# AKGWSB/EzRT

Measured on NVIDIA H100. Metric: Mrays/s (primary+secondary), higher is better.
Workload: dtype f32

## Files before the change

### ezrt_b200/_lib.py

```python
import ctypes as C
import os

from . import build as _build

c_float_p = C.POINTER(C.c_float)
c_int32_p = C.POINTER(C.c_int32)
c_uint32_p = C.POINTER(C.c_uint32)


class RenderParams(C.Structure):
    _fields_ = [
        ("width", C.c_int32), ("height", C.c_int32), ("spp", C.c_int32), ("first_frame", C.c_uint32),
        ("max_bounce", C.c_int32), ("mode", C.c_int32),
        ("eye", C.c_float * 3), ("camera_rotate", C.c_float * 16), ("env_color", C.c_float * 3),
        ("traverse", C.c_int32), ("pipeline", C.c_int32), ("out_channels", C.c_int32),
        ("part_rank", C.c_int32), ("part_count", C.c_int32), ("frames_per_batch", C.c_int32),
        ("profile", C.c_int32), ("reserved", C.c_int32 * 3),
    ]


class AdaptiveParams(C.Structure):
    _fields_ = [("threshold", C.c_float), ("min_spp", C.c_int32), ("check_interval", C.c_int32), ("reserved", C.c_int32)]


# ... 7 lines not shown
                ("reserved", C.c_int32)]


class Counters(C.Structure):
    _fields_ = [
        ("rays", C.c_uint64), ("primary_rays", C.c_uint64), ("bounce_rays", C.c_uint64), ("shadow_rays", C.c_uint64),
        ("samples", C.c_uint64), ("kernel_launches", C.c_uint64), ("device_ms", C.c_double),
        ("deferred_rays", C.c_uint64), ("node_visits", C.c_uint64), ("tri_tests", C.c_uint64), ("node_visits_96", C.c_uint64),
        ("node_bytes", C.c_uint64), ("tri_bytes", C.c_uint64),
    ]


SIGNATURES = {
    "ezrt_last_error": (C.c_char_p, []),
    "ezrt_version": (C.c_int, []),
    "ezrt_scene_create": (C.c_int, [C.c_int, c_float_p, C.c_int, c_float_p, C.c_int, c_float_p, c_float_p, C.c_int, C.c_int,
                                    C.c_int, C.POINTER(C.c_void_p)]),
    "ezrt_scene_destroy": (C.c_int, [C.c_void_p]),
    "ezrt_scene_set_medium": (C.c_int, [C.c_void_p, C.POINTER(Medium)]),
    "ezrt_render": (C.c_int, [C.c_void_p, C.POINTER(RenderParams), c_float_p]),
    "ezrt_render_device": (C.c_int, [C.c_void_p, C.POINTER(RenderParams), C.c_void_p, C.c_void_p]),
    "ezrt_render_adaptive_device": (C.c_int, [C.c_void_p, C.POINTER(RenderParams), C.POINTER(AdaptiveParams), C.c_void_p, C.c_void_p,
                                              C.c_void_p, C.c_void_p]),
    "ezrt_render_adaptive": (C.c_int, [C.c_void_p, C.POINTER(RenderParams), C.POINTER(AdaptiveParams), c_float_p, c_int32_p, c_float_p]),
    "ezrt_render_aov_device": (C.c_int, [C.c_void_p, C.POINTER(RenderParams), C.c_void_p, C.c_void_p, C.c_void_p, C.c_void_p]),
    "ezrt_render_aov": (C.c_int, [C.c_void_p, C.POINTER(RenderParams), c_float_p, c_float_p, c_float_p]),
    "ezrt_denoise_device": (C.c_int, [C.c_void_p, C.POINTER(DenoiseParams), C.c_void_p, C.c_int, C.c_void_p, C.c_void_p, C.c_int, C.c_int,
                                      C.c_int, C.c_void_p, C.c_void_p]),
    "ezrt_denoise": (C.c_int, [C.c_void_p, C.POINTER(DenoiseParams), c_float_p, C.c_int, c_float_p, c_float_p, C.c_int, C.c_int, C.c_int,
                               c_float_p]),
    "ezrt_get_counters": (C.c_int, [C.c_void_p, C.POINTER(Counters)]),
    "ezrt_get_kernel_times": (C.c_int, [C.c_void_p, C.POINTER(C.c_double), C.POINTER(C.c_uint64)]),
    "ezrt_get_w8_phase_cycles": (C.c_int, [C.c_void_p, C.POINTER(C.c_uint64)]),
    "ezrt_partition_pixels": (C.c_int64, [C.c_int, C.c_int, C.c_int, C.c_int]),
    "ezrt_partition_scatter": (C.c_int, [C.c_void_p, C.c_void_p, C.c_int, C.c_int, C.c_int, C.c_int, C.c_int, C.c_void_p]),
    "ezrt_partition_cache_clear": (C.c_int, [C.c_int]),
    "ezrt_host_sort_is_reference": (C.c_int, []),
    "ezrt_accel_build": (C.c_int, [C.c_int, c_float_p, C.c_int, C.c_int, C.c_int, c_int32_p, c_float_p, C.c_int, c_uint32_p, C.POINTER(C.c_double)]),
    "ezrt_partition_scatter_host": (C.c_int, [c_float_p, c_float_p, C.c_int, C.c_int, C.c_int, C.c_int, C.c_int]),
    "ezrt_trace_rays": (C.c_int, [C.c_void_p, C.c_int, c_float_p, c_float_p, C.c_int, C.c_int, C.c_int, c_int32_p, c_float_p,
                                  c_int32_p, c_int32_p, c_float_p, c_float_p]),
    "ezrt_scene_lights": (C.c_int, [C.c_void_p, C.c_int, c_int32_p, c_float_p, C.POINTER(C.c_double)]),
    "ezrt_scene_env_light": (C.c_int, [C.c_void_p, c_float_p, c_float_p, c_float_p, C.POINTER(C.c_double)]),
    "ezrt_occluded_rays": (C.c_int, [C.c_void_p, C.c_int, c_float_p, c_float_p, c_float_p, C.c_int, c_int32_p]),
    "ezrt_eval_brdf": (C.c_int, [C.c_int, C.c_int, C.c_int, c_float_p, c_float_p, c_float_p, c_float_p, c_float_p, c_float_p]),
    "ezrt_eval_bsdf": (C.c_int, [C.c_int, C.c_int, C.c_int, c_float_p, c_float_p, c_float_p, c_float_p, c_int32_p, c_float_p, c_float_p]),
    "ezrt_camera_rays": (C.c_int, [C.c_void_p, C.POINTER(RenderParams), C.c_int, c_uint32_p, c_uint32_p, c_uint32_p, c_float_p, c_float_p]),
    "ezrt_eval_math": (C.c_int, [C.c_int, C.c_int, C.c_int, c_float_p, c_float_p, c_float_p]),
    "ezrt_post_tonemap": (C.c_int, [C.c_void_p, C.c_int, C.c_void_p, C.c_int64, C.c_float, C.c_void_p]),
    "ezrt_write_png": (C.c_int, [C.c_char_p, c_float_p, C.c_int, C.c_int, C.c_int, C.c_int]),
    "ezrt_trilist_create": (C.c_void_p, []),
    "ezrt_trilist_destroy": (None, [C.c_void_p]),
    "ezrt_trilist_size": (C.c_int, [C.c_void_p]),
    "ezrt_transform_matrix": (None, [c_float_p, c_float_p, c_float_p, c_float_p]),
    "ezrt_trilist_read_obj": (C.c_int, [C.c_void_p, C.c_char_p, c_float_p, c_float_p, C.c_int]),
    "ezrt_trilist_read_obj_text": (C.c_int, [C.c_void_p, C.c_char_p, C.c_size_t, c_float_p, c_float_p, C.c_int]),
    "ezrt_trilist_append_encoded": (C.c_int, [C.c_void_p, c_float_p, C.c_int]),
    "ezrt_trilist_build_bvh": (C.c_int, [C.c_void_p, C.c_int, C.c_int]),
    "ezrt_trilist_node_count": (C.c_int, [C.c_void_p]),
    "ezrt_trilist_encode_triangles": (C.c_int, [C.c_void_p, c_float_p]),
    "ezrt_trilist_encode_nodes": (C.c_int, [C.c_void_p, c_float_p]),
    "ezrt_scene_file_load": (C.c_int, [C.c_char_p, C.c_void_p, c_float_p, C.c_char_p, C.c_size_t]),
    "ezrt_hdr_load": (C.c_int, [C.c_char_p, C.POINTER(C.c_int), C.POINTER(C.c_int), c_float_p]),
    "ezrt_hdr_cache": (C.c_int, [c_float_p, C.c_int, C.c_int, c_float_p]),
    "ezrt_hdr_cache_device": (C.c_int, [C.c_int, c_float_p, C.c_int, C.c_int, c_float_p, C.POINTER(C.c_double)]),
    "ezrt_camera_orbit": (None, [C.c_float, C.c_float, C.c_float, c_float_p, c_float_p]),
# ... 38 lines not shown
```

### ezrt_b200/api.py

```python
import ctypes as C
from dataclasses import dataclass, field

import numpy as np

from . import _lib
from ._lib import AdaptiveParams, Counters, DenoiseParams, EzrtError, Medium, RenderParams, check, lib

MODE_DIFFUSE_P3 = 0
MODE_DISNEY_ANISO_P4 = 1
MODE_DISNEY_SOBOL_P5 = 2
MODE_DISNEY_IS_MIS_P5 = 3
MODE_DISNEY_LIGHTS = 4
PARAM_ACCUMULATE = 1
PARAM_ENV_LIGHT = 2
PARAM_TRANSMISSION = 4
PARAM_THIN_LENS = 8
PARAM_MEDIUM = 16
MODES = {"diffuse_p3": 0, "disney_aniso_p4": 1, "disney_sobol_p5": 2, "disney_is_mis_p5": 3, "disney_lights": 4}

TRAVERSE_ACCEL = 0
TRAVERSE_REFERENCE = 1
TRAVERSE_PRUNED = 2
PIPELINE_WAVEFRONT = 0
PIPELINE_MEGAKERNEL = 1
# ... 325 lines not shown
        feat, m2 = _f32(aov, (h, w, AOV_CHANNELS)), _f32(luma2, (h, w))
        if out is None:
            out = np.empty_like(img)
        assert out.dtype == np.float32 and out.shape == img.shape and out.flags.c_contiguous
        d = denoise_params(**{**DENOISE_DEFAULTS, **sigmas})
        check(lib.ezrt_denoise(self._h, C.byref(d), _fp(img), ch, _fp(feat), _fp(m2), w, h, int(n), _fp(out)))
        return out

    def denoise_device(self, d_image, channels, d_aov, d_luma2, width, height, n, d_out, stream=None, **sigmas):
        ptr = lambda t: t.data_ptr() if hasattr(t, "data_ptr") else int(t)
        st = 0 if stream is None else (stream.cuda_stream if hasattr(stream, "cuda_stream") else int(stream))
        d = denoise_params(**{**DENOISE_DEFAULTS, **sigmas})
        check(lib.ezrt_denoise_device(self._h, C.byref(d), C.c_void_p(ptr(d_image)), int(channels), C.c_void_p(ptr(d_aov)),
                                      C.c_void_p(ptr(d_luma2)), int(width), int(height), int(n), C.c_void_p(ptr(d_out)), C.c_void_p(st)))
        return d_out

    def counters(self):
        c = Counters()
        check(lib.ezrt_get_counters(self._h, C.byref(c)))
        return c

    def kernel_times(self):
        ms = (C.c_double * 4)()
        n = (C.c_uint64 * 4)()
        check(lib.ezrt_get_kernel_times(self._h, ms, n))
        return {k: (ms[i], int(n[i])) for i, k in enumerate(("extend", "shade", "shadow", "other"))}

    def w8_phase_cycles(self):
        c = (C.c_uint64 * 8)()
        check(lib.ezrt_get_w8_phase_cycles(self._h, c))
        phases = ("refill", "node", "triangle", "ray_end")
        return {k: {ph: int(c[4 * i + j]) for j, ph in enumerate(phases)} for i, k in enumerate(("k_extend_w8", "k_shadow_w8"))}

    def trace_rays(self, origins, dirs, traverse=TRAVERSE_ACCEL, any_hit=False, p3_normal_fudge=False):
        o = _f32(origins, (-1, 3))
        d = _f32(dirs, (-1, 3))
        n = o.shape[0]
        hit = np.zeros(n, dtype=np.int32); tri = np.zeros(n, dtype=np.int32); inside = np.zeros(n, dtype=np.int32)
        dist = np.zeros(n, dtype=np.float32); point = np.zeros((n, 3), dtype=np.float32); normal = np.zeros((n, 3), dtype=np.float32)
        ip = lambda a: a.ctypes.data_as(_lib.c_int32_p)
        check(lib.ezrt_trace_rays(self._h, n, _fp(o), _fp(d), int(traverse), int(bool(any_hit)), int(bool(p3_normal_fudge)),
                                  ip(hit), _fp(dist), ip(tri), ip(inside), _fp(point), _fp(normal)))
        return dict(hit=hit, distance=dist, triangle=tri, inside=inside, point=point, normal=normal)

    def camera_rays(self, cfg, px, py, frame):
        u = lambda a: np.ascontiguousarray(a, dtype=np.uint32).reshape(-1)
        px, py, frame = u(px), u(py), u(frame)
        n = px.size
        assert py.size == n and frame.size == n
        o, d = np.zeros((n, 3), np.float32), np.zeros((n, 3), np.float32)
        p = cfg.to_struct()
        up = lambda a: a.ctypes.data_as(_lib.c_uint32_p)
        check(lib.ezrt_camera_rays(self._h, C.byref(p), n, up(px), up(py), up(frame), _fp(o), _fp(d)))
        return o, d

    def lights(self):
        k = check(lib.ezrt_scene_lights(self._h, 0, None, None, None))
        tri = np.zeros(k, np.int32)
        cdf = np.zeros(k, np.float32)
        total = C.c_double(0.0)
        check(lib.ezrt_scene_lights(self._h, k, tri.ctypes.data_as(_lib.c_int32_p), _fp(cdf), C.byref(total)))
        return tri, cdf, total.value

    def env_light_table(self):
        total = C.c_double(0.0)
        if not check(lib.ezrt_scene_env_light(self._h, None, None, None, C.byref(total))):
# ... 78 lines not shown
```

### ezrt_b200/csrc/accel_w8.cpp

```cpp
#include <math.h>
#include <sched.h>
#include <stdio.h>
#include <stdlib.h>
#include <string.h>

#include <algorithm>
#include <atomic>
#include <chrono>
#include <thread>
#include <utility>
#include <vector>

#include "ezrt_internal.h"
#include "w8_node.h"

namespace {

inline float box_area(const EzrtAccelNode& c) {
    const float x = c.BB[0] - c.AA[0], y = c.BB[1] - c.AA[1], z = c.BB[2] - c.AA[2];
    return x * y + x * z + y * z;
}

}

// ... 138 lines not shown
    Pick stack[32];
    int sp = 0;
    stack[sp++] = {n0, k0};
    while (sp > 0) {
        Pick p = stack[--sp];
        const float* c = &C[(size_t)p.n * 8];
        while (p.k > 1 && c[p.k] == c[p.k - 1]) p.k--;
        if (p.k == 1 || a[p.n].n > 0) { roots[cnt++] = p.n; continue; }
        const EzrtAccelNode& nd = a[p.n];
        const float *cl = &C[(size_t)nd.left * 8], *cr = &C[(size_t)nd.right * 8];
        int bk = 1;
        float best = 3.0e38f;
        for (int k = 1; k < p.k; k++)
            if (cl[k] + cr[p.k - k] < best) { best = cl[k] + cr[p.k - k]; bk = k; }
        stack[sp++] = {nd.right, p.k - bk};
        stack[sp++] = {nd.left, bk};
    }
    return cnt;
}

int EzrtCollapse::children(int b, int* ch) const {
    const std::vector<EzrtAccelNode>& a = *an;
    const EzrtAccelNode& nd = a[b];
    const float *cl = &C[(size_t)nd.left * 8], *cr = &C[(size_t)nd.right * 8];
    int bk = 1;
    float best = 3.0e38f;
    for (int k = 1; k <= width - 1; k++)
        if (cl[k] + cr[width - k] < best) { best = cl[k] + cr[width - k]; bk = k; }
    int cnt = collect(nd.left, bk, ch);
    cnt += collect(nd.right, width - bk, ch + cnt);
    return cnt;
}

#define W8_COST_NODE 1.0
#define W8_COST_TRI 0.4

int ezrt_build_w8(const std::vector<EzrtAccelNode>& an, const std::vector<uint32_t>& order_in, float pad, float max_abs_coord,
                  const int axis_bit[3], EzrtW8Tree& out) {
    out.nodes.clear();
    out.tri_order.clear();
    out.leaf_first.assign(an.size(), -1);
    out.depth = 0;
    out.n_nodes = 0;
    out.n_children = 0;
    if (an.empty()) return -1;
    const int NB = (int)an.size();
    const double min_step = (double)max_abs_coord * (double)W8_MIN_STEP_REL;
    EzrtCollapse col;
    const int crc = col.build(an, 8, W8_MAX_LEAF_TRIS, W8_COST_NODE, W8_COST_TRI);
    if (crc) return crc;
    const std::vector<int>& first = col.first;
    const std::vector<int>& count = col.count;
    const std::vector<char>& as_leaf = col.as_leaf;

    struct Item { int bnode, level; };
    std::vector<Item> queue;
    queue.push_back({0, 1});
    out.tri_order.reserve(order_in.size());
    std::vector<int> new_pos(order_in.size(), -1);
    for (size_t wi = 0; wi < queue.size(); wi++) {
        const int b = queue[wi].bnode, level = queue[wi].level;
        out.depth = std::max(out.depth, level);
        int ch[8];
        int cnt = 0;
        if (an[b].n > 0 || (wi == 0 && as_leaf[b])) {
            ch[cnt++] = b;
        } else {
            cnt = col.children(b, ch);
        }
        double nlo[3] = {3.0e38, 3.0e38, 3.0e38}, nhi[3] = {-3.0e38, -3.0e38, -3.0e38};
        for (int k = 0; k < cnt; k++)
            for (int a = 0; a < 3; a++) {
                nlo[a] = std::min(nlo[a], (double)an[ch[k]].AA[a] - (double)pad);
                nhi[a] = std::max(nhi[a], (double)an[ch[k]].BB[a] + (double)pad);
            }
        int slot_child[8];
        for (int s = 0; s < 8; s++) slot_child[s] = -1;
        {
            double cost[8][8];
            for (int k = 0; k < cnt; k++)
                for (int s = 0; s < 8; s++) {
                    double c = 0.0;
// ... 340 lines not shown
```

### ezrt_b200/csrc/capi.cu

```cuda
#include <cuda_runtime.h>

#include <chrono>
#include <cmath>
#include <cstdio>
#include <cstdlib>
#include <cstring>
#include <functional>
#include <array>
#include <map>
#include <mutex>
#include <new>
#include <string>
#include <thread>
#include <vector>

#include "device_scene.h"
#include "ezrt.h"
#include "ezrt_internal.h"
#include "ezrt_math.h"
#include "kernels.h"
#include "w8_node.h"

#define CU_CHECK(call)                                                                                  \
    do {                                                                                                \
// ... 531 lines not shown
            return ezrt_set_error(EZRT_ERR_CUDA, "scene_create: upload failed: %s", cudaGetErrorString(cudaGetLastError()));
    }
    lap("triangles: upload");
    EzrtPrepInfo prep;
    {
        int r = sc->tri_geo.ensure((size_t)n_triangles * 4 * sizeof(float4));
        if (!r) r = sc->tri_shade.ensure((size_t)n_triangles * 3 * sizeof(float4));
        if (!r) r = ezrt_prep_records((const float*)raw.p, n_triangles, sc->tri_geo.p, sc->tri_shade.p, prep);
        if (r) return r;
    }
    std::vector<float4> mats;
    for (int m = 0; m < prep.n_materials; m++) {
        const float* v = &prep.materials[(size_t)m * EZRT_MATERIAL_FLOATS];
        mats.push_back(make_float4(v[0], v[1], v[2], v[3]));
        mats.push_back(make_float4(v[4], v[5], v[6], v[7]));
        mats.push_back(make_float4(v[8], v[9], v[10], v[11]));
        mats.push_back(make_float4(v[12], v[13], v[14], v[15]));
        mats.push_back(make_float4(v[16], v[17], 0.0f, 0.0f));
    }
    const float max_abs = prep.max_abs;
    float bmin[3], bmax[3];
    for (int k = 0; k < 3; k++) { bmin[k] = prep.bmin[k]; bmax[k] = prep.bmax[k]; }
    lap("triangles: geometry / shading records, materials (device)");
    const float prune_delta = max_abs * 1.52587890625e-05f;
    EzrtW4Tree w4;
    EzrtRawArray<float>& acc_wide = w4.nodes;
    EzrtRawArray<uint32_t>& acc_wide_q = w4.q16;
    std::vector<uint32_t> w8_words;
    int acc_wide_root = 0;
    std::vector<uint32_t> acc_order;
    int acc_depth = 0, w8_depth = 0, w8_near_bit[3] = {0, 1, 2};
    bool have_accel = true;
    {
        std::vector<EzrtAccelNode> an;
        std::vector<uint32_t> order_bin;
        const char* be = getenv("EZRT_BUILD");
        if (be && !strcmp(be, "host")) {
            ezrt_build_accel(tris, n_triangles, W8_MAX_LEAF_TRIS, an, order_bin);
            lap("acceleration tree: binary SAH build (host)");
        } else {
            const int brc = ezrt_build_accel_device((const float*)raw.p, n_triangles, W8_MAX_LEAF_TRIS, an, order_bin, nullptr);
            if (brc < 0) return brc;
            lap("acceleration tree: binary SAH build (device)");
        }
        const float pad = 2.0f * prune_delta;
        int accel_form = (n_triangles >= (1 << 16)) ? 8 : 4;
        if (const char* we = getenv("EZRT_ACCEL")) {
            const int v = atoi(we);
            if (v == 4 || v == 8) accel_form = v;
        }
        if (an[0].n > 0) accel_form = 8;
        EzrtW8Tree w8;
        ezrt_w8_axis_bits(bmin, bmax, w8_near_bit);
        if (accel_form == 8) {
            const int wrc = ezrt_build_w8(an, order_bin, pad, max_abs, w8_near_bit, w8);
            if (wrc != 0 || w8.depth > EZRT_W8_SMEM_STACK + W8_LOCAL_STACK) {
                have_accel = false;
            } else {
                acc_order = w8.tri_order;
                w8_words.swap(w8.nodes);
                w8_depth = w8.depth;
            }
        } else {
            const char* ce = getenv("EZRT_W4_COLLAPSE");
            const bool greedy = ce && !strcmp(ce, "greedy");
            const char* qe = getenv("EZRT_ACCEL_Q16");
            const bool want_q16 = !(qe && atoi(qe) == 0);
            if (ezrt_build_w4(an, pad, max_abs, greedy, want_q16, ezrt_host_threads(), w4) != 0) {
                have_accel = false;
            } else {
                acc_order = order_bin;
                acc_wide_root = w4.root;
                acc_depth = w4.depth;
                if (3 * w4.depth + 2 > EZRT_ACCEL_STACK) { w4.nodes.clear(); have_accel = false; }
                if (!have_accel) w4.q16.clear();
            }
        }
        if (!have_accel) {
            acc_order.resize(n_triangles);
            for (int i = 0; i < n_triangles; i++) acc_order[i] = (uint32_t)i;
        }
        raw.release();
    }
    lap("acceleration tree: collapse, pack");
    if (guard.worker.joinable()) guard.worker.join();
    if (verbose) fprintf(stderr, "[ezrt_scene_create] %-44s %8.1f ms (worker thread, overlapped)\n", "reference tree: decode, validate, repack", ref_ms);
    if (ref_rc) return ezrt_set_error(ref_rc, "%s", ref_msg.c_str());
    lap("wait for the reference-tree worker");
// ... 672 lines not shown
    CU_CHECK(cudaMemcpyAsync(d_aov, aov, sizeof(float) * 8 * npix, cudaMemcpyHostToDevice, st));
    CU_CHECK(cudaMemcpyAsync(d_color, color, sizeof(float) * channels * npix, cudaMemcpyHostToDevice, st));
    CU_CHECK(cudaMemcpyAsync(d_luma2, luma2, sizeof(float) * npix, cudaMemcpyHostToDevice, st));
    if ((rc = denoise_impl(s, dp, d_color, channels, d_aov, d_luma2, width, height, n_frames, d_color, st))) return rc;
    CU_CHECK(cudaMemcpyAsync(out, d_color, sizeof(float) * channels * npix, cudaMemcpyDeviceToHost, st));
    CU_CHECK(cudaStreamSynchronize(st));
    return EZRT_OK;
}

int ezrt_get_counters(ezrt_scene* s, ezrt_counters* out) {
    if (!s || !out) return ezrt_set_error(EZRT_ERR_INVALID, "get_counters: null argument");
    memset(out, 0, sizeof(*out));
    if (!s->have_timing) return EZRT_OK;
    CU_CHECK(cudaSetDevice(s->device));
    CU_CHECK(cudaEventSynchronize(s->ev_stop));
    unsigned long long t[8] = {0, 0, 0, 0, 0, 0, 0, 0};
    CU_CHECK(cudaMemcpy(t, s->totals_buf.p, sizeof(t), cudaMemcpyDeviceToHost));
    out->deferred_rays = t[4];
    out->node_visits = t[5] + t[7];
    out->tri_tests = t[6];
    out->node_bytes = t[5] * 128ull + t[7] * 96ull;
    out->tri_bytes = t[6] * 64ull;
    out->node_visits_96 = t[7];
    float ms = 0.0f;
    CU_CHECK(cudaEventElapsedTime(&ms, s->ev_start, s->ev_stop));
    out->primary_rays = t[0]; out->bounce_rays = t[1]; out->shadow_rays = t[2];
    out->rays = t[0] + t[1] + t[2];
    out->samples = t[3];
    out->kernel_launches = s->launches;
    out->device_ms = ms;
    return EZRT_OK;
}

int ezrt_get_w8_phase_cycles(ezrt_scene* s, uint64_t* out) {
    if (!s || !out) return ezrt_set_error(EZRT_ERR_INVALID, "get_w8_phase_cycles: null argument");
    for (int k = 0; k < 8; k++) out[k] = 0;
    if (!s->have_timing) return EZRT_OK;
    CU_CHECK(cudaSetDevice(s->device));
    CU_CHECK(cudaEventSynchronize(s->ev_stop));
    static_assert(EZRT_W8_PHASES_SHADOW == EZRT_W8_PHASES_EXTEND + 4 && 5 + EZRT_W8_PHASES_SHADOW + 4 <= EZRT_TOTALS, "totals layout");
    CU_CHECK(cudaMemcpy(out, (unsigned long long*)s->totals_buf.p + 5 + EZRT_W8_PHASES_EXTEND, sizeof(uint64_t) * 8, cudaMemcpyDeviceToHost));
    return EZRT_OK;
}

int ezrt_get_kernel_times(ezrt_scene* s, double* ms, uint64_t* launches) {
    if (!s || !ms || !launches) return ezrt_set_error(EZRT_ERR_INVALID, "get_kernel_times: null argument");
    for (int k = 0; k < 4; k++) { ms[k] = 0.0; launches[k] = 0; }
    if (!s->have_timing || s->spans.empty()) return EZRT_OK;
    CU_CHECK(cudaSetDevice(s->device));
    CU_CHECK(cudaEventSynchronize(s->ev_stop));
    for (const auto& sp : s->spans) {
        float t = 0.0f;
        CU_CHECK(cudaEventElapsedTime(&t, s->ev_pool[sp.e0], s->ev_pool[sp.e1]));
        ms[sp.cls] += t;
        launches[sp.cls] += 1;
    }
    return EZRT_OK;
}

int64_t ezrt_partition_pixels(int width, int height, int rank, int count) {
    if (width <= 0 || height <= 0 || count < 1 || rank < 0 || rank >= count) return EZRT_ERR_INVALID;
    int64_t n = 0;
    for (const TileDev& t : partition_tiles(width, height, rank, count)) n += (int64_t)t.w * t.h;
    return n;
}

int ezrt_partition_scatter(const float* d_compact, float* d_full, int width, int height, int channels, int rank, int count,
                           void* cuda_stream) {
    if (!d_compact || !d_full || channels < 1) return ezrt_set_error(EZRT_ERR_INVALID, "partition_scatter: bad argument");
    if (width <= 0 || height <= 0 || count < 1 || rank < 0 || rank >= count) return ezrt_set_error(EZRT_ERR_INVALID, "partition_scatter: bad partition");
    auto& cache = scatter_cache();
    std::mutex& mu = scatter_mutex();
    int device = 0;
    CU_CHECK(cudaGetDevice(&device));
    cudaStream_t st = (cudaStream_t)cuda_stream;
// ... 348 lines not shown
```

### ezrt_b200/csrc/device_functions.cuh

```cuda
#ifndef EZRT_DEVICE_FUNCTIONS_CUH
#define EZRT_DEVICE_FUNCTIONS_CUH

#include "device_scene.h"
#include "ezrt.h"
#include "ezrt_math.h"
#include "w8_node.h"

__constant__ uint32_t c_sobolV[8 * 32] = {
#include "ezrt_sobol_table.inc"
};

typedef ez_vec3 vec3;

__device__ __forceinline__ vec3 f4xyz(float4 q) { return ez_v3(q.x, q.y, q.z); }
__device__ __forceinline__ vec3 splat3(float s) { return ez_v3(s, s, s); }
__device__ __forceinline__ float4 ldg4(const float4* p) { return __ldg(p); }

#ifndef EZRT_MATH_NOINLINE
#define EZRT_MATH_NOINLINE 0
#endif
#if EZRT_MATH_NOINLINE
#define EZD_MATH __device__ __noinline__
#else
#define EZD_MATH __device__ __forceinline__
// ... 793 lines not shown

#define W8_ENDED (-2)
template <bool ANYHIT, bool COUNT, bool IDX, bool BOUNDED = false, class RayIO>
__device__ __forceinline__ void extend_w8(const SceneDev& sc, uint32_t n, uint32_t* work, RayIO io, const unsigned char* s_perm, uint2* stack_sm,
                                          W8Counts counts, unsigned long long* phase_cycles) {
    const bool tri_na = sc.tri_l1_bypass != 0;
    const int refill_thresh = sc.refill_thresh, leaf_thresh = sc.w8_tri_weight;
    const unsigned FULL = 0xffffffffu;
    const int lane = threadIdx.x & 31;
    const unsigned lt_mask = (1u << lane) - 1u;
    const int stack_stride = blockDim.x;
    const int stack_cap = sc.w8_stack_entries;
    uint2 stack_local[W8_LOCAL_STACK];
    uint2* const my_stack = stack_sm + threadIdx.x;
    const uint4* __restrict__ nodes = sc.w8_nodes;
    const float origin_limit = sc.w8_origin_limit, inv_limit = sc.quant_inv_limit;
    const uint32_t bias = sc.w8_decode_bits;
    __shared__ unsigned char s_owner_all[EZRT_EXTEND_MAX_THREADS];
    unsigned char* const s_owner = s_owner_all + (threadIdx.x & ~31u);

    int ray = -1;
    int node = -1;
    int end_leaf = 0;
    int sp = 0;
    vec3 o = splat3(0.0f), d = splat3(0.0f), inv = splat3(0.0f);
    float slack = 0.0f, best = EZ_INF;
    int best_tri = -1;
    bool tie = false;
    uint32_t near_mask = 0;
    uint32_t g_base = 0, g_bits = 0;
    uint32_t t_base = 0, t_mask = 0;
    uint32_t n_visits = 0, n_tests = 0;
    uint32_t cyc_refill = 0, cyc_node = 0, cyc_tri = 0, cyc_end = 0;
    uint32_t end_dt = 0, t_mark = COUNT ? w8_clock() : 0u;
    bool exhausted = false;
    uint32_t chunk_pos = 0, chunk_end = 0;
    const uint32_t chunk = (uint32_t)sc.work_chunk;

#define W8_PUSH(e) do { const uint2 e__ = (e); if (sp < stack_cap) my_stack[sp * stack_stride] = e__; else stack_local[sp - stack_cap] = e__; ++sp; } while (0)
#define W8_POP() ((--sp < stack_cap) ? my_stack[sp * stack_stride] : stack_local[sp - stack_cap])
    auto select_next = [&]() {
        if ((g_bits >> 8) == 0u) {
            if (sp == 0) {
                const uint32_t te = COUNT ? w8_clock() : 0u;
                if (best_tri >= 0) end_leaf = io.leaf_of(best_tri);
                if (COUNT) end_dt = w8_clock() - te;
                node = W8_ENDED;
                return;
            }
            const uint2 e = W8_POP();
            g_base = e.x;
            g_bits = e.y;
        }
        const int p = 23 - __clz(g_bits);
        g_bits ^= 0x100u << p;
        const uint32_t slot = (uint32_t)p ^ near_mask;
        node = (int)(g_base + __popc(g_bits & 0xffu & ((1u << slot) - 1u)));
    };

    while (true) {
        const bool ended = node == W8_ENDED;
        const unsigned need = __ballot_sync(FULL, ray < 0 || ended);
        const bool claim = need != 0u && !exhausted && chunk_pos >= chunk_end;
        uint32_t base = 0;
        if (claim && lane == 0) base = atomicAdd(work, chunk);
        if (ended) {
// ... 156 lines not shown
                    unsigned mn = tb;
#pragma unroll
                    for (int s = 1; s < 32; s <<= 1) {
                        const unsigned v = __shfl_down_sync(FULL, mn, s);
                        if (lane + s < end) mn = min(mn, v);
                    }
                    const unsigned run_min = __shfl_sync(FULL, mn, start);
                    const unsigned win = __ballot_sync(FULL, act && tb != 0xffffffffu && tb == run_min) & seg;
                    const int p = win ? __ffs(win) - 1 : lane;
                    const int triw = __shfl_sync(FULL, tri, p);
                    const float tn = __uint_as_float(__shfl_sync(FULL, tb, p));
                    if (win) {
                        if (tn < best) {
                            best = tn;
                            best_tri = triw;
                            tie = __popc(win) > 1;
                        } else {
                            tie = true;
                        }
                    }
                }
                const int k_last = __shfl_sync(FULL, k, 31);
                if (owns) {
                    t_mask = (taken < cnt && !stop) ? t_mask & ~((2u << k_last) - 1u) : 0u;
                    if (stop) { g_bits = 0u; sp = 0; }
                    if (t_mask == 0u) select_next();
                }
            }
            busy = __ballot_sync(FULL, ray >= 0 && node != W8_ENDED);
            if (COUNT) {
                const uint32_t now = w8_clock(), e = __reduce_max_sync(FULL, end_dt);
                end_dt = 0u;
                cyc_end += e;
                if (node_step) cyc_node += now - t_mark - e;
                else cyc_tri += now - t_mark - e;
                t_mark = now;
            }
        } while (busy != 0u && (exhausted || __popc(busy) >= refill_thresh));
    }
#undef W8_PUSH
#undef W8_POP
    if (COUNT) {
        atomicAdd(counts.node_visits, (unsigned long long)n_visits);
        atomicAdd(counts.tri_tests, (unsigned long long)n_tests);
        if (lane == 0) {
            atomicAdd(phase_cycles + 0, (unsigned long long)cyc_refill);
            atomicAdd(phase_cycles + 1, (unsigned long long)cyc_node);
            atomicAdd(phase_cycles + 2, (unsigned long long)cyc_tri);
            atomicAdd(phase_cycles + 3, (unsigned long long)cyc_end);
        }
    }
}

template <int K>
__device__ __forceinline__ float warp_reduce_f(float v) {
#pragma unroll
    for (int s = 16; s > 0; s >>= 1) {
        const float u = __shfl_xor_sync(0xffffffffu, v, s);
        v = K ? fmaxf(v, u) : fminf(v, u);
    }
    return v;
}
__device__ __forceinline__ void w8_bundle_axis(float lo, float hi, uint32_t sign, const float4 b, float& entry, float& exit) {
    const float omin = b.x, omax = b.y, vmin = b.z, vmax = b.w;
    const bool pos = sign == 1u;
    const float pn = pos ? lo : hi, pf = pos ? hi : lo;
    const float xe = pos ? __fsub_rd(pn, omax) : __fsub_ru(pn, omin);
    const float xx = pos ? __fsub_ru(pf, omin) : __fsub_rd(pf, omax);
    entry = sign ? __fmul_rd(xe, xe >= 0.0f ? vmin : vmax) : -EZ_INF;
    exit = sign ? __fmul_ru(xx, xx >= 0.0f ? vmax : vmin) : EZ_INF;
}

template <bool COUNT, bool IDX, class RayIO>
__device__ __forceinline__ void extend_w8_bundle(const SceneDev& sc, uint32_t n, uint32_t* work, RayIO io, const unsigned char* s_perm, uint2* stack_sm,
                                                 W8Counts counts) {
    const bool tri_na = sc.tri_l1_bypass != 0;
    const unsigned FULL = 0xffffffffu;
    const int lane = threadIdx.x & 31;
    uint2* const stack = stack_sm + (threadIdx.x >> 5) * W8_BUNDLE_STACK;
    __shared__ float4 s_bnd_all[(EZRT_EXTEND_MAX_THREADS / 32) * 3];
    float4* const bnd = s_bnd_all + (threadIdx.x >> 5) * 3;
    __shared__ unsigned s_pend_all[EZRT_EXTEND_MAX_THREADS / 32];
// ... 835 lines not shown
```

### ezrt_b200/csrc/ezrt_internal.h

```cpp
#ifndef EZRT_INTERNAL_H
#define EZRT_INTERNAL_H

#include "ezrt.h"

#ifdef __cplusplus
extern "C" {
#endif

int ezrt_set_error(int code, const char* fmt, ...)
#if defined(__GNUC__)
    __attribute__((format(printf, 2, 3)))
#endif
    ;

#ifdef __cplusplus
}
#endif

#ifdef __cplusplus
#include <stdint.h>
#include <stdio.h>
#include <stdlib.h>

#include <chrono>
// ... 55 lines not shown
                     void* d_acc_shade, int* d_acc_leaf, uint32_t* d_ref_to_acc);
int ezrt_prep_vertex_ids(const void* d_acc_geo, int n, uint32_t* d_vid, uint32_t* d_vert_src, int& n_vert);
int ezrt_prep_indexed(const void* d_acc_geo, int n, const uint32_t* d_vid, const uint32_t* d_vert_src, int n_vert, void* d_rec, void* d_vert);

struct EzrtCollapse {
    const std::vector<EzrtAccelNode>* an = nullptr;
    int width = 0;
    std::vector<int> first, count;
    std::vector<char> as_leaf;
    EzrtRawArray<float> C;
    int build(const std::vector<EzrtAccelNode>& an, int width, int max_leaf, double cost_node, double cost_tri, int threads = 1);
    int collect(int n0, int k0, int* roots) const;
    int children(int b, int* ch) const;
};

struct EzrtW4Tree {
    EzrtRawArray<float> nodes;
    EzrtRawArray<uint32_t> q16;
    int root = 0, depth = 0;
    EzrtCollapse col;
};
int ezrt_build_w4(const std::vector<EzrtAccelNode>& an, float pad, float max_abs_coord, bool greedy, bool want_q16, int threads, EzrtW4Tree& out);

struct EzrtW8Tree {
    std::vector<uint32_t> nodes;
    std::vector<uint32_t> tri_order;
    std::vector<int> leaf_first;
    int depth;
    int n_nodes;
    long long n_children;
};
void ezrt_w8_axis_bits(const float bmin[3], const float bmax[3], int axis_bit[3]);
int ezrt_build_w8(const std::vector<EzrtAccelNode>& an, const std::vector<uint32_t>& order_in, float pad, float max_abs_coord,
                  const int axis_bit[3], EzrtW8Tree& out);

float ezrt_quant_inv_limit(double max_scale, double bias, float max_abs_coord);
float ezrt_w8_max_scale(const uint32_t* nodes, size_t n_nodes);
float ezrt_q16_max_scale(const uint32_t* nodes, size_t n_nodes);
#endif

#define EZRT_PART_TILE 16

#endif
```

### ezrt_b200/csrc/kernels.h

```cpp
#ifndef EZRT_KERNELS_H
#define EZRT_KERNELS_H

#include <algorithm>

#include "device_scene.h"

#ifndef EZRT_EXTEND_MAX_THREADS
#define EZRT_EXTEND_MAX_THREADS 1024
#endif
#define EZRT_EXTEND_THREADS EZRT_EXTEND_MAX_THREADS
#ifndef EZRT_EXTEND_LB_BLOCKS
#define EZRT_EXTEND_LB_BLOCKS 1
#endif
#define EZRT_EXTEND_BLOCKS_PER_SM 1

struct LightOptions {
    LightsDev lights{};
    EnvDev env{};
    MediumDev med{};
    bool env_on = false, trans_on = false, medium_on = false;
};

void launch_generate(const RenderDev& rd, const TileDev* tiles, uint32_t n_slots, uint32_t batch_first_frame, PathQueue q,
                     uint32_t* q_count, int n_sms, cudaStream_t st, const LensDev* lens = nullptr);
void launch_extend(const SceneDev& sc, bool prune, bool anyhit, PathQueue q, const uint32_t* q_count, uint32_t* work,
                   const uint32_t* perm, int to_accel, uint32_t n_max, int n_sms, cudaStream_t st, float2* side_hit = nullptr, int gate = 0);
#define EZRT_W8_PHASES_EXTEND 3
#define EZRT_W8_PHASES_SHADOW 7
#define EZRT_TOTALS 16
void launch_extend_accel(const SceneDev& sc, PathQueue q, const uint32_t* q_count, uint32_t* work, uint32_t* defer_list,
                         uint32_t* defer_count, uint32_t* defer_work, uint32_t n_max, int n_sms, unsigned long long* counts, const uint32_t* perm,
                         cudaStream_t st, int exact_gate = 0);
void launch_ray_sort(const SceneDev& sc, PathQueue q, const uint32_t* q_count, uint32_t* keys, uint32_t* bins, uint32_t* perm,
                     uint32_t n_max, int n_sms, cudaStream_t st);
void launch_shadow(const SceneDev& sc, bool prune, ShadowQueue sq, const uint32_t* s_count, uint32_t* work, float4* Lo,
                   const uint32_t* perm, uint32_t n_max, int n_sms, cudaStream_t st, bool bounded = false);
void launch_shadow_accel(const SceneDev& sc, ShadowQueue sq, const uint32_t* s_count, uint32_t* work, float4* Lo, uint32_t* defer_list,
                         uint32_t* defer_count, uint32_t* defer_work, uint32_t n_max, int n_sms, unsigned long long* counts, cudaStream_t st,
                         bool bounded = false);
void launch_shade(const SceneDev& sc, const RenderDev& rd, const TileDev* tiles, int bounce, uint32_t batch_first_frame,
                  PathQueue qin, const uint32_t* in_count, PathQueue qout, uint32_t* out_count, ShadowQueue sq,
                  uint32_t* s_count, float4* Lo, float4* Le, uint32_t n_max, uint32_t n_fused, uint32_t n_frames, int n_sms, cudaStream_t st,
                  float4* aov_rec,
                  const LightOptions& o);
void launch_extend_camera(const SceneDev& sc, const RenderDev& rd, const TileDev* tiles, uint32_t batch_first_frame, uint32_t n_slots, uint32_t n_frames, PathQueue q,
                          uint32_t* work, uint32_t* defer_list, uint32_t* defer_count, uint32_t* defer_work, int n_sms, unsigned long long* counts,
                          cudaStream_t st, int exact_gate = 0);
void launch_deferred_lane(const SceneDev& sc, const RenderDev& rd, const TileDev* tiles, int bounce, uint32_t batch_first_frame, PathQueue qin,
                          const uint32_t* defer_list, const uint32_t* defer_count, uint32_t* defer_work, float2* side_hit, PathQueue qout,
                          uint32_t* out_count, ShadowQueue sq, uint32_t* s_count, float4* Lo, float4* Le, uint32_t n_fused, uint32_t n_frames,
                          int n_sms, cudaStream_t st, float4* aov_rec, const LightOptions& o);
void launch_nee(const SceneDev& sc, const RenderDev& rd, ShadowQueue sq, const uint32_t* s_count, float4* Lo, uint32_t n_max, int n_sms, cudaStream_t st,
                const LightOptions& o);
void launch_light_weights(const SceneDev& sc, float* w, cudaStream_t st);
void launch_env_weights(const SceneDev& sc, float* w, cudaStream_t st);
void launch_light_compact(const float* w, int n, int32_t* idx_out, float* w_out, int32_t* count, cudaStream_t st);
void launch_light_records(const SceneDev& sc, const int32_t* idx, int n, float4* rec, cudaStream_t st);
void launch_blend(const RenderDev& rd, const TileDev* tiles, int nf, uint32_t batch_first_frame, const float4* Lo, const float4* Le,
                  float* fb, float* luma2, int32_t* spp_map, const float4* aov_rec, float* aov, cudaStream_t st);
void launch_adaptive_check(const RenderDev& rd, const TileDev* tiles_in, int n_frames, float threshold, const float* fb, const float* luma2,
                           unsigned char* keep, unsigned int* blocks_done, TileDev* tiles_out, int32_t* counts, cudaStream_t st);
void launch_tally(const uint32_t* q_counts, const uint32_t* s_counts, const uint32_t* d_ext, const uint32_t* d_sh, int n_stages,
// ... 20 lines not shown
```

### ezrt_b200/csrc/w8_node.h

```cpp
#ifndef EZRT_W8_NODE_H
#define EZRT_W8_NODE_H

#include <stdint.h>

#define W8_NODE_WORDS 20
#define W8_NODE_BYTES 80
#define W8_MAX_LEAF_TRIS 4
#define W8_MAX_NODE_TRIS 32
#define W8_SLACK_STEPS 0.25
#define W8_DECODE_BIAS 32768.0f
#define W8_DECODE_BITS 0x47000000u
#define W8_MIN_STEP_REL 7.62939453125e-06f
#define W8_ORIGIN_LIMIT_REL 4.0f
#define W8_INV_LIMIT 7.9228162514264338e28f
#define W8_INV_MIN 8.6736173798840355e-19f

#define W8_LOCAL_STACK 48
#define W8_BUNDLE_STACK 64

#define W8_W_ORIGIN 0
#define W8_W_EXP_IMASK 3
#define W8_W_CHILD_BASE 4
#define W8_W_TRI_BASE 5
#define W8_W_QLO 6
#define W8_W_META 12
#define W8_W_QHI 14

#define W8_SCALE_BITS(w, a) ((((uint32_t)(w) >> (8 * (a))) & 0xffu) << 23)

#endif
```

### include/ezrt.h

```cpp
#ifndef EZRT_H
#define EZRT_H

#include <stddef.h>
#include <stdint.h>

#ifdef __cplusplus
extern "C" {
#endif

#define EZRT_TRIANGLE_FLOATS 36
#define EZRT_BVHNODE_FLOATS 12
#define EZRT_MATERIAL_FLOATS 18

typedef enum ezrt_status {
    EZRT_OK = 0,
    EZRT_ERR_INVALID = -1,
    EZRT_ERR_IO = -2,
    EZRT_ERR_CUDA = -3,
    EZRT_ERR_BAD_TREE = -4,
    EZRT_ERR_NOMEM = -5
} ezrt_status;

typedef enum ezrt_mode {
    EZRT_MODE_DIFFUSE_P3 = 0,
// ... 82 lines not shown
    int32_t min_spp;
    int32_t check_interval;
    int32_t reserved;
} ezrt_adaptive_params;

int ezrt_render_adaptive_device(ezrt_scene* scene, const ezrt_render_params* params, const ezrt_adaptive_params* adaptive,
                                float* d_framebuffer, int32_t* d_spp, float* d_luma2, void* cuda_stream);
int ezrt_render_adaptive(ezrt_scene* scene, const ezrt_render_params* params, const ezrt_adaptive_params* adaptive,
                         float* framebuffer, int32_t* spp, float* luma2);

int ezrt_render_aov_device(ezrt_scene* scene, const ezrt_render_params* params, float* d_framebuffer, float* d_aov, float* d_luma2,
                           void* cuda_stream);
int ezrt_render_aov(ezrt_scene* scene, const ezrt_render_params* params, float* framebuffer, float* aov, float* luma2);

typedef struct ezrt_denoise_params {
    int32_t iterations;
    float sigma_l;
    float sigma_n;
    float sigma_z;
    float sigma_a;
    int32_t reserved;
} ezrt_denoise_params;

int ezrt_denoise_device(ezrt_scene* scene, const ezrt_denoise_params* params, const float* d_color, int channels, const float* d_aov,
                        const float* d_luma2, int width, int height, int n_frames, float* d_out, void* cuda_stream);
int ezrt_denoise(ezrt_scene* scene, const ezrt_denoise_params* params, const float* color, int channels, const float* aov,
                 const float* luma2, int width, int height, int n_frames, float* out);

int ezrt_get_counters(ezrt_scene* scene, ezrt_counters* out);

int ezrt_get_kernel_times(ezrt_scene* scene, double* ms, uint64_t* launches);

int ezrt_get_w8_phase_cycles(ezrt_scene* scene, uint64_t* out);

int64_t ezrt_partition_pixels(int width, int height, int rank, int count);
int ezrt_partition_scatter(const float* d_compact, float* d_full, int width, int height, int channels,
                           int rank, int count, void* cuda_stream);
int ezrt_partition_cache_clear(int device);
int ezrt_partition_scatter_host(const float* compact, float* full, int width, int height, int channels,
                                int rank, int count);

int ezrt_trace_rays(ezrt_scene* scene, int n, const float* origins, const float* dirs, int traverse,
                    int any_hit, int p3_normal_fudge, int32_t* out_hit, float* out_distance,
                    int32_t* out_triangle, int32_t* out_inside, float* out_point, float* out_normal);

int ezrt_scene_lights(ezrt_scene* scene, int cap, int32_t* tri_out, float* cdf_out, double* total_out);

int ezrt_scene_env_light(ezrt_scene* scene, float* row_cdf, float* col_cdf, float* texel_pdf, double* total);

int ezrt_occluded_rays(ezrt_scene* scene, int n, const float* origins, const float* dirs, const float* tmax, int traverse,
                       int32_t* out_lit);

int ezrt_eval_brdf(int device, int which, int n, const float* V, const float* N, const float* L,
                   const float* xi, const float* materials, float* out);

int ezrt_eval_bsdf(int device, int which, int n, const float* V, const float* N, const float* L, const float* xi,
                   const int32_t* inside, const float* materials, float* out);

int ezrt_camera_rays(ezrt_scene* scene, const ezrt_render_params* params, int n, const uint32_t* px, const uint32_t* py,
                     const uint32_t* frame, float* origins_out, float* dirs_out);

int ezrt_eval_math(int device, int which, int n, const float* a, const float* b, float* out);

int ezrt_accel_build(int device, const float* tris, int n_triangles, int leaf_n, int where, int32_t* links_out,
                     float* boxes_out, int nodes_cap, uint32_t* order_out, double* ms);

// ... 51 lines not shown
```

Measured before the change: 3332.

## Build binary BVH with single-triangle leaves before 8-wide collapse; add step counters

When the 8-wide tree is chosen, the binary SAH build now uses one triangle per leaf instead of four, so the collapse step has full freedom to form its own leaves by SAH cost. The collapse gains a thread-count parameter so it can run multithreaded, and the triangle cost is moved to a shared constant. It also adds per-warp node/triangle step counters and an API to read them under the COUNT path. Risks are a longer build and a different tree quality, which changes traversal cost.

```diff
diff --git a/ezrt_b200/_lib.py b/ezrt_b200/_lib.py
--- a/ezrt_b200/_lib.py
+++ b/ezrt_b200/_lib.py
@@ -63,6 +63,7 @@
     "ezrt_get_counters": (C.c_int, [C.c_void_p, C.POINTER(Counters)]),
     "ezrt_get_kernel_times": (C.c_int, [C.c_void_p, C.POINTER(C.c_double), C.POINTER(C.c_uint64)]),
     "ezrt_get_w8_phase_cycles": (C.c_int, [C.c_void_p, C.POINTER(C.c_uint64)]),
+    "ezrt_get_w8_step_counts": (C.c_int, [C.c_void_p, C.POINTER(C.c_uint64)]),
     "ezrt_partition_pixels": (C.c_int64, [C.c_int, C.c_int, C.c_int, C.c_int]),
     "ezrt_partition_scatter": (C.c_int, [C.c_void_p, C.c_void_p, C.c_int, C.c_int, C.c_int, C.c_int, C.c_int, C.c_void_p]),
     "ezrt_partition_cache_clear": (C.c_int, [C.c_int]),
diff --git a/ezrt_b200/api.py b/ezrt_b200/api.py
--- a/ezrt_b200/api.py
+++ b/ezrt_b200/api.py
@@ -381,6 +381,12 @@
         phases = ("refill", "node", "triangle", "ray_end")
         return {k: {ph: int(c[4 * i + j]) for j, ph in enumerate(phases)} for i, k in enumerate(("k_extend_w8", "k_shadow_w8"))}
 
+    def w8_step_counts(self):
+        c = (C.c_uint64 * 8)()
+        check(lib.ezrt_get_w8_step_counts(self._h, c))
+        names = ("node_steps", "triangle_steps", "node_visits", "triangle_tests")
+        return {k: {nm: int(c[4 * i + j]) for j, nm in enumerate(names)} for i, k in enumerate(("k_extend_w8", "k_shadow_w8"))}
+
     def trace_rays(self, origins, dirs, traverse=TRAVERSE_ACCEL, any_hit=False, p3_normal_fudge=False):
         o = _f32(origins, (-1, 3))
         d = _f32(dirs, (-1, 3))
diff --git a/ezrt_b200/csrc/accel_w8.cpp b/ezrt_b200/csrc/accel_w8.cpp
--- a/ezrt_b200/csrc/accel_w8.cpp
+++ b/ezrt_b200/csrc/accel_w8.cpp
@@ -194,11 +194,8 @@
     return cnt;
 }
 
-#define W8_COST_NODE 1.0
-#define W8_COST_TRI 0.4
-
 int ezrt_build_w8(const std::vector<EzrtAccelNode>& an, const std::vector<uint32_t>& order_in, float pad, float max_abs_coord,
-                  const int axis_bit[3], EzrtW8Tree& out) {
+                  const int axis_bit[3], double cost_tri, int threads, EzrtW8Tree& out) {
     out.nodes.clear();
     out.tri_order.clear();
     out.leaf_first.assign(an.size(), -1);
@@ -209,7 +206,7 @@
     const int NB = (int)an.size();
     const double min_step = (double)max_abs_coord * (double)W8_MIN_STEP_REL;
     EzrtCollapse col;
-    const int crc = col.build(an, 8, W8_MAX_LEAF_TRIS, W8_COST_NODE, W8_COST_TRI);
+    const int crc = col.build(an, 8, W8_MAX_LEAF_TRIS, 1.0, cost_tri, threads);
     if (crc) return crc;
     const std::vector<int>& first = col.first;
     const std::vector<int>& count = col.count;
diff --git a/ezrt_b200/csrc/capi.cu b/ezrt_b200/csrc/capi.cu
--- a/ezrt_b200/csrc/capi.cu
+++ b/ezrt_b200/csrc/capi.cu
@@ -587,28 +587,29 @@
     int acc_depth = 0, w8_depth = 0, w8_near_bit[3] = {0, 1, 2};
     bool have_accel = true;
     {
+        int accel_form = (n_triangles >= (1 << 16)) ? 8 : 4;
+        if (const char* we = getenv("EZRT_ACCEL")) {
+            const int v = atoi(we);
+            if (v == 4 || v == 8) accel_form = v;
+        }
+        if (n_triangles <= W8_MAX_LEAF_TRIS) accel_form = 8;
+        const int leaf_n = (accel_form == 8) ? W8_BINARY_LEAF_TRIS : W8_MAX_LEAF_TRIS;
         std::vector<EzrtAccelNode> an;
         std::vector<uint32_t> order_bin;
         const char* be = getenv("EZRT_BUILD");
         if (be && !strcmp(be, "host")) {
-            ezrt_build_accel(tris, n_triangles, W8_MAX_LEAF_TRIS, an, order_bin);
+            ezrt_build_accel(tris, n_triangles, leaf_n, an, order_bin);
             lap("acceleration tree: binary SAH build (host)");
         } else {
-            const int brc = ezrt_build_accel_device((const float*)raw.p, n_triangles, W8_MAX_LEAF_TRIS, an, order_bin, nullptr);
+            const int brc = ezrt_build_accel_device((const float*)raw.p, n_triangles, leaf_n, an, order_bin, nullptr);
             if (brc < 0) return brc;
             lap("acceleration tree: binary SAH build (device)");
         }
         const float pad = 2.0f * prune_delta;
-        int accel_form = (n_triangles >= (1 << 16)) ? 8 : 4;
-        if (const char* we = getenv("EZRT_ACCEL")) {
-            const int v = atoi(we);
-            if (v == 4 || v == 8) accel_form = v;
-        }
-        if (an[0].n > 0) accel_form = 8;
         EzrtW8Tree w8;
         ezrt_w8_axis_bits(bmin, bmax, w8_near_bit);
         if (accel_form == 8) {
-            const int wrc = ezrt_build_w8(an, order_bin, pad, max_abs, w8_near_bit, w8);
+            const int wrc = ezrt_build_w8(an, order_bin, pad, max_abs, w8_near_bit, W8_COST_TRI, ezrt_host_threads(), w8);
             if (wrc != 0 || w8.depth > EZRT_W8_SMEM_STACK + W8_LOCAL_STACK) {
                 have_accel = false;
             } else {
@@ -1347,15 +1348,29 @@
     return EZRT_OK;
 }
 
-int ezrt_get_w8_phase_cycles(ezrt_scene* s, uint64_t* out) {
-    if (!s || !out) return ezrt_set_error(EZRT_ERR_INVALID, "get_w8_phase_cycles: null argument");
+static int w8_pass_words(ezrt_scene* s, int first, uint64_t* out) {
     for (int k = 0; k < 8; k++) out[k] = 0;
     if (!s->have_timing) return EZRT_OK;
     CU_CHECK(cudaSetDevice(s->device));
     CU_CHECK(cudaEventSynchronize(s->ev_stop));
-    static_assert(EZRT_W8_PHASES_SHADOW == EZRT_W8_PHASES_EXTEND + 4 && 5 + EZRT_W8_PHASES_SHADOW + 4 <= EZRT_TOTALS, "totals layout");
-    CU_CHECK(cudaMemcpy(out, (unsigned long long*)s->totals_buf.p + 5 + EZRT_W8_PHASES_EXTEND, sizeof(uint64_t) * 8, cudaMemcpyDeviceToHost));
-    return EZRT_OK;
+    static_assert(5 + EZRT_W8_PHASES_SHADOW + EZRT_W8_PASS_WORDS <= EZRT_TOTALS, "totals layout");
+    unsigned long long t[EZRT_TOTALS];
+    CU_CHECK(cudaMemcpy(t, s->totals_buf.p, sizeof(t), cudaMemcpyDeviceToHost));
+    for (int k = 0; k < 4; k++) {
+        out[k] = t[5 + EZRT_W8_PHASES_EXTEND + first + k];
+        out[4 + k] = t[5 + EZRT_W8_PHASES_SHADOW + first + k];
+    }
+    return EZRT_OK;
+}
+
+int ezrt_get_w8_phase_cycles(ezrt_scene* s, uint64_t* out) {
+    if (!s || !out) return ezrt_set_error(EZRT_ERR_INVALID, "get_w8_phase_cycles: null argument");
+    return w8_pass_words(s, 0, out);
+}
+
+int ezrt_get_w8_step_counts(ezrt_scene* s, uint64_t* out) {
+    if (!s || !out) return ezrt_set_error(EZRT_ERR_INVALID, "get_w8_step_counts: null argument");
+    return w8_pass_words(s, 4, out);
 }
 
 int ezrt_get_kernel_times(ezrt_scene* s, double* ms, uint64_t* launches) {
diff --git a/ezrt_b200/csrc/device_functions.cuh b/ezrt_b200/csrc/device_functions.cuh
--- a/ezrt_b200/csrc/device_functions.cuh
+++ b/ezrt_b200/csrc/device_functions.cuh
@@ -849,6 +849,7 @@
     uint32_t t_base = 0, t_mask = 0;
     uint32_t n_visits = 0, n_tests = 0;
     uint32_t cyc_refill = 0, cyc_node = 0, cyc_tri = 0, cyc_end = 0;
+    uint32_t n_node_steps = 0, n_tri_steps = 0;
     uint32_t end_dt = 0, t_mark = COUNT ? w8_clock() : 0u;
     bool exhausted = false;
     uint32_t chunk_pos = 0, chunk_end = 0;
@@ -1071,8 +1072,8 @@
                 const uint32_t now = w8_clock(), e = __reduce_max_sync(FULL, end_dt);
                 end_dt = 0u;
                 cyc_end += e;
-                if (node_step) cyc_node += now - t_mark - e;
-                else cyc_tri += now - t_mark - e;
+                if (node_step) { cyc_node += now - t_mark - e; n_node_steps++; }
+                else { cyc_tri += now - t_mark - e; n_tri_steps++; }
                 t_mark = now;
             }
         } while (busy != 0u && (exhausted || __popc(busy) >= refill_thresh));
@@ -1082,11 +1083,15 @@
     if (COUNT) {
         atomicAdd(counts.node_visits, (unsigned long long)n_visits);
         atomicAdd(counts.tri_tests, (unsigned long long)n_tests);
+        atomicAdd(phase_cycles + 6, (unsigned long long)n_visits);
+        atomicAdd(phase_cycles + 7, (unsigned long long)n_tests);
         if (lane == 0) {
             atomicAdd(phase_cycles + 0, (unsigned long long)cyc_refill);
             atomicAdd(phase_cycles + 1, (unsigned long long)cyc_node);
             atomicAdd(phase_cycles + 2, (unsigned long long)cyc_tri);
             atomicAdd(phase_cycles + 3, (unsigned long long)cyc_end);
+            atomicAdd(phase_cycles + 4, (unsigned long long)n_node_steps);
+            atomicAdd(phase_cycles + 5, (unsigned long long)n_tri_steps);
         }
     }
 }
diff --git a/ezrt_b200/csrc/ezrt_internal.h b/ezrt_b200/csrc/ezrt_internal.h
--- a/ezrt_b200/csrc/ezrt_internal.h
+++ b/ezrt_b200/csrc/ezrt_internal.h
@@ -111,7 +111,7 @@
 };
 void ezrt_w8_axis_bits(const float bmin[3], const float bmax[3], int axis_bit[3]);
 int ezrt_build_w8(const std::vector<EzrtAccelNode>& an, const std::vector<uint32_t>& order_in, float pad, float max_abs_coord,
-                  const int axis_bit[3], EzrtW8Tree& out);
+                  const int axis_bit[3], double cost_tri, int threads, EzrtW8Tree& out);
 
 float ezrt_quant_inv_limit(double max_scale, double bias, float max_abs_coord);
 float ezrt_w8_max_scale(const uint32_t* nodes, size_t n_nodes);
diff --git a/ezrt_b200/csrc/kernels.h b/ezrt_b200/csrc/kernels.h
--- a/ezrt_b200/csrc/kernels.h
+++ b/ezrt_b200/csrc/kernels.h
@@ -25,9 +25,10 @@
                      uint32_t* q_count, int n_sms, cudaStream_t st, const LensDev* lens = nullptr);
 void launch_extend(const SceneDev& sc, bool prune, bool anyhit, PathQueue q, const uint32_t* q_count, uint32_t* work,
                    const uint32_t* perm, int to_accel, uint32_t n_max, int n_sms, cudaStream_t st, float2* side_hit = nullptr, int gate = 0);
+#define EZRT_W8_PASS_WORDS 8
 #define EZRT_W8_PHASES_EXTEND 3
-#define EZRT_W8_PHASES_SHADOW 7
-#define EZRT_TOTALS 16
+#define EZRT_W8_PHASES_SHADOW (EZRT_W8_PHASES_EXTEND + EZRT_W8_PASS_WORDS)
+#define EZRT_TOTALS 24
 void launch_extend_accel(const SceneDev& sc, PathQueue q, const uint32_t* q_count, uint32_t* work, uint32_t* defer_list,
                          uint32_t* defer_count, uint32_t* defer_work, uint32_t n_max, int n_sms, unsigned long long* counts, const uint32_t* perm,
                          cudaStream_t st, int exact_gate = 0);
diff --git a/ezrt_b200/csrc/w8_node.h b/ezrt_b200/csrc/w8_node.h
--- a/ezrt_b200/csrc/w8_node.h
+++ b/ezrt_b200/csrc/w8_node.h
@@ -7,6 +7,8 @@
 #define W8_NODE_BYTES 80
 #define W8_MAX_LEAF_TRIS 4
 #define W8_MAX_NODE_TRIS 32
+#define W8_BINARY_LEAF_TRIS 1
+#define W8_COST_TRI 0.4
 #define W8_SLACK_STEPS 0.25
 #define W8_DECODE_BIAS 32768.0f
 #define W8_DECODE_BITS 0x47000000u
diff --git a/include/ezrt.h b/include/ezrt.h
--- a/include/ezrt.h
+++ b/include/ezrt.h
@@ -138,6 +138,7 @@
 int ezrt_get_kernel_times(ezrt_scene* scene, double* ms, uint64_t* launches);
 
 int ezrt_get_w8_phase_cycles(ezrt_scene* scene, uint64_t* out);
+int ezrt_get_w8_step_counts(ezrt_scene* scene, uint64_t* out);
 
 int64_t ezrt_partition_pixels(int width, int height, int rank, int count);
 int ezrt_partition_scatter(const float* d_compact, float* d_full, int width, int height, int channels,
```

Result: faster. 3524, median of 6 (+5.8%).
